# facebookresearch/gtn_applications

Hardware: AMD Instinct MI355X
Metric: utterances/sec fwd+bwd (ctc_benchmark T=1000,C=100,B=128); HBM GB/s vs peak (higher is better)
Workload: dtype f32

## Files before the change

gtn_applications_amd/csrc/ctc_kernels.hip:

```cpp
#include <atomic>
#include <string>
#include <type_traits>

#include "device_common.h"

#ifndef WFL_MITM_STATS
#define WFL_MITM_STATS 0
#endif

namespace wfl {

constexpr float kNegBig = -1.0e30f;
constexpr float kLog2e = 1.4426950408889634f;
constexpr int kBlk = 16;

__device__ __forceinline__ float lse2_b2(float a, float b) {
  const float e = __builtin_amdgcn_exp2f(-fabsf(a - b));
  return vmax(a, b) + __builtin_amdgcn_logf(1.f + e);
}
__device__ __forceinline__ float readlane_f(float v, int lane) {
  return __int_as_float(__builtin_amdgcn_readlane(__float_as_int(v), lane));
}
__device__ __forceinline__ float to_score(float raw) {
  const float v = raw * kLog2e;
// ... 358 lines not shown
  "s_nop 1\n\t"  \
  "v_cndmask_b32_e64 %[t0], %[v1], %[v0], %[m0]\n\t"  \
  "v_cndmask_b32_e64 %[t1], %[v0], %[v1], %[m0]\n\t"  \
  "v_cndmask_b32_e64 %[t2], %[v3], %[v2], %[m0]\n\t"  \
  "v_cndmask_b32_e64 %[t3], %[v2], %[v3], %[m0]\n\t"  \
  OP " %[a0], %[t0], %[t1] quad_perm:[1,0,3,2] row_mask:0xf bank_mask:0xf\n\t"  \
  "v_cndmask_b32_e64 %[t0], %[v5], %[v4], %[m0]\n\t"  \
  "v_cndmask_b32_e64 %[t1], %[v4], %[v5], %[m0]\n\t"  \
  OP " %[a1], %[t2], %[t3] quad_perm:[1,0,3,2] row_mask:0xf bank_mask:0xf\n\t"  \
  "v_cndmask_b32_e64 %[t2], %[v7], %[v6], %[m0]\n\t"  \
  "v_cndmask_b32_e64 %[t3], %[v6], %[v7], %[m0]\n\t"  \
  OP " %[a2], %[t0], %[t1] quad_perm:[1,0,3,2] row_mask:0xf bank_mask:0xf\n\t"  \
  "v_cndmask_b32_e64 %[t0], %[v9], %[v8], %[m0]\n\t"  \
  "v_cndmask_b32_e64 %[t1], %[v8], %[v9], %[m0]\n\t"  \
  OP " %[a3], %[t2], %[t3] quad_perm:[1,0,3,2] row_mask:0xf bank_mask:0xf\n\t"  \
  "v_cndmask_b32_e64 %[t2], %[v11], %[v10], %[m0]\n\t"  \
  "v_cndmask_b32_e64 %[t3], %[v10], %[v11], %[m0]\n\t"  \
  OP " %[a4], %[t0], %[t1] quad_perm:[1,0,3,2] row_mask:0xf bank_mask:0xf\n\t"  \
  "v_cndmask_b32_e64 %[t0], %[v13], %[v12], %[m0]\n\t"  \
  "v_cndmask_b32_e64 %[t1], %[v12], %[v13], %[m0]\n\t"  \
  OP " %[a5], %[t2], %[t3] quad_perm:[1,0,3,2] row_mask:0xf bank_mask:0xf\n\t"  \
  "v_cndmask_b32_e64 %[t2], %[v15], %[v14], %[m0]\n\t"  \
  "v_cndmask_b32_e64 %[t3], %[v14], %[v15], %[m0]\n\t"  \
  OP " %[a6], %[t0], %[t1] quad_perm:[1,0,3,2] row_mask:0xf bank_mask:0xf\n\t"  \
  "s_nop 0\n\t"  \
  OP " %[a7], %[t2], %[t3] quad_perm:[1,0,3,2] row_mask:0xf bank_mask:0xf\n\t"  \
  "v_cndmask_b32_e64 %[t0], %[a1], %[a0], %[m1]\n\t"  \
  "v_cndmask_b32_e64 %[t1], %[a0], %[a1], %[m1]\n\t"  \
  "v_cndmask_b32_e64 %[t2], %[a3], %[a2], %[m1]\n\t"  \
  "v_cndmask_b32_e64 %[t3], %[a2], %[a3], %[m1]\n\t"  \
  OP " %[a0], %[t0], %[t1] quad_perm:[2,3,0,1] row_mask:0xf bank_mask:0xf\n\t"  \
  "v_cndmask_b32_e64 %[t0], %[a5], %[a4], %[m1]\n\t"  \
  "v_cndmask_b32_e64 %[t1], %[a4], %[a5], %[m1]\n\t"  \
  OP " %[a2], %[t2], %[t3] quad_perm:[2,3,0,1] row_mask:0xf bank_mask:0xf\n\t"  \
  "v_cndmask_b32_e64 %[t2], %[a7], %[a6], %[m1]\n\t"  \
  "v_cndmask_b32_e64 %[t3], %[a6], %[a7], %[m1]\n\t"  \
  OP " %[a4], %[t0], %[t1] quad_perm:[2,3,0,1] row_mask:0xf bank_mask:0xf\n\t"  \
  "s_nop 0\n\t"  \
  OP " %[a6], %[t2], %[t3] quad_perm:[2,3,0,1] row_mask:0xf bank_mask:0xf\n\t"  \
  OP " %[a1], %[a0], %[a0] row_ror:12 row_mask:0xf bank_mask:0x5\n\t"  \
  OP " %[a1], %[a2], %[a2] row_ror:12 row_mask:0xf bank_mask:0xa\n\t"  \
  OP " %[a3], %[a4], %[a4] row_ror:12 row_mask:0xf bank_mask:0x5\n\t"  \
  OP " %[a3], %[a6], %[a6] row_ror:12 row_mask:0xf bank_mask:0xa\n\t"  \
  "s_nop 1\n\t"  \
  OP " %[a0], %[a1], %[a1] row_ror:8 row_mask:0xf bank_mask:0x3\n\t"  \
  OP " %[a0], %[a3], %[a3] row_ror:8 row_mask:0xf bank_mask:0xc"
template <bool MAX>
__device__ __forceinline__ float fold16(const float (&v)[16], int lane) {
  float a0, a1, a2, a3, a4, a5, a6, a7, t0, t1, t2, t3;
  const unsigned long long m0 = 0xaaaaaaaaaaaaaaaaull, m1 = 0xccccccccccccccccull;
#define WFL_FOLD16_OPERANDS                                                                                             \
  : [a0] "=&v"(a0), [a1] "=&v"(a1), [a2] "=&v"(a2), [a3] "=&v"(a3), [a4] "=&v"(a4), [a5] "=&v"(a5), [a6] "=&v"(a6),    \
    [a7] "=&v"(a7), [t0] "=&v"(t0), [t1] "=&v"(t1), [t2] "=&v"(t2), [t3] "=&v"(t3)                                      \
  : [v0] "v"(v[0]), [v1] "v"(v[1]), [v2] "v"(v[2]), [v3] "v"(v[3]), [v4] "v"(v[4]), [v5] "v"(v[5]), [v6] "v"(v[6]),    \
    [v7] "v"(v[7]), [v8] "v"(v[8]), [v9] "v"(v[9]), [v10] "v"(v[10]), [v11] "v"(v[11]), [v12] "v"(v[12]),              \
    [v13] "v"(v[13]), [v14] "v"(v[14]), [v15] "v"(v[15]), [m0] "s"(m0), [m1] "s"(m1)
  if (MAX)
    asm(WFL_FOLD16_BODY("v_max_f32_dpp") WFL_FOLD16_OPERANDS);
  else
    asm(WFL_FOLD16_BODY("v_add_f32_dpp") WFL_FOLD16_OPERANDS);
#undef WFL_FOLD16_OPERANDS
  typedef unsigned v2u __attribute__((ext_vector_type(2)));
  v2u sw = __builtin_amdgcn_permlane16_swap(__float_as_uint(a0), __float_as_uint(a0), false, false);
  float t = MAX ? vmax(__uint_as_float(sw.x), __uint_as_float(sw.y)) : __uint_as_float(sw.x) + __uint_as_float(sw.y);
  sw = __builtin_amdgcn_permlane32_swap(__float_as_uint(t), __float_as_uint(t), false, false);
  t = MAX ? vmax(__uint_as_float(sw.x), __uint_as_float(sw.y)) : __uint_as_float(sw.x) + __uint_as_float(sw.y);
  return t;
}
__device__ __forceinline__ float fold16_sum(const float (&v)[16], int lane) { return fold16<false>(v, lane); }

typedef __attribute__((address_space(3))) int lds_int_t;
__device__ __forceinline__ int lds_peek(const int* p) { return *(const volatile lds_int_t*)(const lds_int_t*)p; }
__device__ __forceinline__ void lds_post(int* p, int v) {
  asm volatile("" ::: "memory");
  *(volatile lds_int_t*)(lds_int_t*)p = v;
}

#define WFL_FRAME(P, PH, TT, TL, TH, F, FY)                                   \
  "v_pk_mul_f32 v[6:7], " F ", %[G]\n\t"                                      \
  "v_pk_mul_f32 " TT ", " F ", " P " op_sel_hi:[1,0]\n\t"                     \
  "v_fmac_f32_dpp " TL ", " PH ", v6 wave_shr:1 row_mask:0xf bank_mask:0xf\n\t" \
  "v_fmac_f32_dpp " TH ", " PH ", v7 wave_shr:1 row_mask:0xf bank_mask:0xf\n\t" \
  "v_fmac_f32 " TH ", " FY ", " PH "\n\t"

__device__ __forceinline__ void lsm_seed_rows(float* rows, const float* __restrict__ xsrc, int n, int C, float lse_blk,
                                              float cf_row, int lane) {
  const int total = n * C;
  const unsigned magic = (unsigned)((0x100000000ull + (unsigned)C - 1) / (unsigned)C);
  auto seed = [&](float xv, float l) {
    const float e = __expf((xv == xv ? xv : WFL_NEG_INF) - l);
    return l > WFL_NEG_INF ? -cf_row * e : 0.f;
  };
  constexpr int U = 8;
  if ((C & 3) == 0 && (((uintptr_t)xsrc) & 15) == 0) {
    const int n4 = total >> 2;
    for (int i0 = lane; i0 < n4; i0 += 64 * U) {
      float4 v[U];
      float l[U];
#pragma unroll
      for (int u = 0; u < U; ++u) {
        const int i = min(i0 + 64 * u, n4 - 1);
        v[u] = ((const float4*)xsrc)[i];
        l[u] = __shfl(lse_blk, (int)__umulhi((unsigned)i * 4u, magic), 64);
      }
#pragma unroll
      for (int u = 0; u < U; ++u) {
        const int i = i0 + 64 * u;
        if (i < n4) ((float4*)rows)[i] = float4{seed(v[u].x, l[u]), seed(v[u].y, l[u]), seed(v[u].z, l[u]), seed(v[u].w, l[u])};
      }
    }
  } else {
    for (int i0 = lane; i0 < total; i0 += 64 * U) {
      float v[U], l[U];
#pragma unroll
      for (int u = 0; u < U; ++u) {
        const int i = min(i0 + 64 * u, total - 1);
        v[u] = xsrc[i];
        l[u] = __shfl(lse_blk, (int)__umulhi((unsigned)i, magic), 64);
      }
#pragma unroll
      for (int u = 0; u < U; ++u) {
        const int i = i0 + 64 * u;
        if (i < total) rows[i] = seed(v[u], l[u]);
      }
    }
  }
}

constexpr int kCS = 65;
constexpr int kCTileBytes = kBlk * kCS * 4;
__host__ __device__ __forceinline__ size_t compact_wave_bytes(int C) { return (size_t)kCTileBytes + ((C + 15) & ~15); }
__device__ __forceinline__ void compact_init(float* tile, unsigned char* cmap, int C, int lane) {
  for (int i = lane; i < kBlk * kCS; i += 64) tile[i] = 0.f;
  for (int i = lane; i < ((C + 15) & ~15) / 4; i += 64) ((unsigned int*)cmap)[i] = 0x40404040u;
}
__device__ __forceinline__ void compact_expand(const float* tile, const unsigned char* cmap, float* __restrict__ dst,
                                               const float* __restrict__ xsrc, float lse_blk, int n, int C, float cf,
                                               bool alive, bool soft, int lane) {
  auto softterm = [&](float xv, float l) { return l > WFL_NEG_INF ? cf * __expf((xv == xv ? xv : WFL_NEG_INF) - l) : 0.f; };
  typedef float f4u __attribute__((ext_vector_type(4), aligned(4)));
  const int c4n = C >> 2;
#pragma unroll 2
  for (int j = 0; j < n; ++j) {
    const float l = soft ? readlane_f(lse_blk, j) : 0.f;
    const float* tr = tile + j * kCS;
    float* drow = dst + (int64_t)j * C;
    const float* xr = xsrc + (int64_t)j * C;
    for (int c4 = lane; c4 < c4n; c4 += 64) {
      const unsigned m4 = alive ? ((const unsigned int*)cmap)[c4] : 0x40404040u;
      f4u o = {tr[m4 & 255u], tr[(m4 >> 8) & 255u], tr[(m4 >> 16) & 255u], tr[m4 >> 24]};
      if (soft) {
        const f4u xv = *reinterpret_cast<const f4u*>(xr + 4 * c4);
        o.x -= softterm(xv.x, l), o.y -= softterm(xv.y, l), o.z -= softterm(xv.z, l), o.w -= softterm(xv.w, l);
      }
      *reinterpret_cast<f4u*>(drow + 4 * c4) = o;
    }
    const int c = 4 * c4n + lane;
    if (c < C) {
      float v = tr[alive ? (int)cmap[c] : 64];
      if (soft) v -= softterm(xr[c], l);
      drow[c] = v;
    }
  }
}

template <bool PIPE, bool LSM = false, bool COMPACT = false>
// ... 1129 lines not shown
```

gtn_applications_amd/csrc/ctc_mitm.h:

```cpp
#pragma once

#ifndef WFL_MITM_ABL
#define WFL_MITM_ABL 0
#endif
#ifndef WFL_MITM_STORE
#define WFL_MITM_STORE 2
#endif
#ifndef WFL_MITM_CLAMP_EVERY
#define WFL_MITM_CLAMP_EVERY 1
#endif
#ifndef WFL_MITM_LEAN
#define WFL_MITM_LEAN 1
#endif
#ifndef WFL_MITM_LSM_ROWS
#define WFL_MITM_LSM_ROWS 8
#endif
constexpr int kLsmRows = WFL_MITM_LSM_ROWS;
#ifndef WFL_MITM_STATS
#define WFL_MITM_STATS 0
#endif

constexpr int kMSpinDefault = 1 << 24;
constexpr int kMaxCouple = 100;
constexpr int kMTile = 128;
// ... 29 lines not shown
      default: role = 4, idx = 7; break;
    }
  }
};
template <>
struct MitmK<8> {
  static constexpr int kSlots = 5, kPSlots = 3;
  static constexpr int kStagers = 2, kEmitters = 3, kWaves = 8;
  __device__ static __forceinline__ void role(int wave, int& role, int& idx) {
    switch (wave) {
      case 0: role = 0, idx = 0; break;
      case 4: role = 2, idx = 0; break;
      case 1: role = 3, idx = 0; break;
      case 2: role = 1, idx = 0; break;
      case 3: role = 1, idx = 1; break;
      case 5: role = 4, idx = 0; break;
      case 6: role = 4, idx = 1; break;
      default: role = 4, idx = 2; break;
    }
  }
};

typedef float mv4f __attribute__((ext_vector_type(4)));
template <class K>
struct MitmLds {
  mv4f ring[K::kSlots][kBlk / 2][64];
  float4 pck[K::kPSlots][64];
  float4 ck[K::kSlots][64];
  float fref[K::kSlots][kBlk];
  double offc[K::kSlots];
  double poff[K::kPSlots];
  double offtot;
  int staged[K::kSlots];
  int pready[K::kPSlots];
  int egrab[K::kSlots];
  int pgrab[K::kPSlots];
  double zref;
  int zready;
  int enext;
  int chainpos;
  int ckpos;
  int ckdone;
  int offdone;
  int cmap_ready;
  int abort;
#if WFL_MITM_STATS
  long long blk_t[64];
#endif
};


template <class K>
__device__ __forceinline__ void mitm_give_up(const CtcArgs& a, const CtcWs& w, MitmLds<K>& S) {
  if ((threadIdx.x & 63) == 0) {
    __hip_atomic_fetch_or((int32_t*)(a.ws + w.perr), 1, __ATOMIC_RELAXED, __HIP_MEMORY_SCOPE_AGENT);
    coherent_store64(a.ws + w.suspect, a.token);
  }
  lds_post(&S.abort, 1);
  asm volatile("s_waitcnt vmcnt(0) lgkmcnt(0)" ::: "memory");
  __builtin_amdgcn_endpgm();
}
template <class K>
__device__ __forceinline__ bool mitm_waited_out(const CtcArgs& a, MitmLds<K>& S, int spin) {
  return spin > a.spin || ((spin & 255) == 255 && lds_peek(&S.abort) != 0);
}

__host__ __device__ inline int mitm_first_emitted(int NB, int dir) { return dir == 0 ? NB / 2 : NB - NB / 2; }
__device__ __forceinline__ unsigned long long* mitm_pub(const CtcArgs& a, const CtcWs& w, int b, int dir, int NB) {
  return (unsigned long long*)(a.ws + w.ck) + (int64_t)(b * 2 + dir) * (NB + 1) * a.P;
}

#if WFL_MITM_STATS
#define MITM_T0() const long long _t0 = clock64()
#define MITM_ACC(var) var += clock64() - _t0
#else
#define MITM_T0()
#define MITM_ACC(var)
#endif

typedef float mv2f __attribute__((ext_vector_type(2)));

template <class K, int DIR, bool FULL, bool WIDE, bool LSM = false>
__device__ __forceinline__ void ctc_mitm_emit_block(const mv2f (&F)[kBlk], mv2f sa, int ea, float4 pk, float rsum, double off_sum,
                                                    MitmLds<K>& S, bool first,
                                                    int cnt, float cf, float g, float gs, bool skipn, bool owner, bool adder,
                                                    int lane, float* rows, const unsigned char* cmap, int ycol, int blank, int C, long long* zmm,
                                                    int32_t* zcnt, unsigned long long* suspect, unsigned long long suspect_token,
                                                    int32_t* perr, int spin_bound, float* __restrict__ dst, long long* st_part,
                                                    const float* __restrict__ xsrc = nullptr, float lse_rows = 0.f) {
#if WFL_MITM_STATS
  const long long st_e0 = clock64();
#endif
  const int eb = __float_as_int(pk.z);
  mv2f pa[kBlk];
  const mv2f G = {g, gs};
#pragma unroll
  for (int j = 0; j < kBlk; ++j) {
    if (FULL || j < cnt) {
      const mv2f t = F[j] * G;
      const mv2f o = F[j] * mv2f{sa.x, sa.x};
      float ox = o.x, oy = o.y;
      fmac2_shr1(ox, oy, sa.y, t.x, t.y);
      oy = fmaf(F[j].y, sa.y, oy);
      sa = mv2f{ox, oy};
    }
    pa[j] = sa;
  }
#if WFL_MITM_STATS
  {
    const long long now = __builtin_amdgcn_readfirstlane(__float_as_int(sa.x)) * 0 + clock64();
    st_part[0] += now - st_e0;
  }
#endif
  float bb = pk.x, bl = pk.y;
  float Kn = 0.f;
  bool alive;
  double zk = -1.0e300;
  const int sx = ea + eb;
  if (first) {
    const int eb_next = __builtin_amdgcn_update_dpp(eb, eb, 0x130, 0xf, 0xf, false);
    const float h = lane == 63 ? 0.f : ldexpf(1.f, min(max(eb_next - eb, -200), 100));
    const float hs = skipn ? h : 0.f;
    const float tb0 = bb + bl;
    float tl0 = bl;
    fmac2_shl1(tl0, bb, bl, h, hs);
    const float v = sa.x * tb0 + sa.y * tl0;
    const int own = v > 0.f ? sx + __builtin_amdgcn_frexp_expf(v) : kEmptyE;
    const int E = __builtin_amdgcn_readlane(wave_prefix_max_i(own), 63);
    const float term = v > 0.f ? ldexpf(v, max(sx - E, -200)) : 0.f;
    const float Zm = wave_all_sum(term);
    alive = Zm > 0.f && Zm < 3.0e38f && E > kEmptyE;
    if (alive) Kn = cf * ldexpf(__builtin_amdgcn_rcpf(Zm), min(max(sx - E, -200), 100));
    zk = alive ? off_sum + (double)E + (double)__builtin_amdgcn_logf(Zm) + (double)rsum : -1.0e300;
    if (lane == 0) S.zref = zk;
    lds_post(&S.zready, 1);
    if (lane == 0) {
      const long long zq = z_fixed(zk);
      const long long was_lo = __hip_atomic_fetch_min(zmm, zq, __ATOMIC_RELAXED, __HIP_MEMORY_SCOPE_AGENT);
      const long long was_hi = __hip_atomic_fetch_max(zmm + 1, zq, __ATOMIC_RELAXED, __HIP_MEMORY_SCOPE_AGENT);
      asm volatile("s_waitcnt vmcnt(0)" ::"v"(was_lo), "v"(was_hi) : "memory");
      __hip_atomic_fetch_add(zcnt, 1, __ATOMIC_RELAXED, __HIP_MEMORY_SCOPE_AGENT);
    }
  } else {
    for (int spin = 0; lds_peek(&S.zready) != 1; ++spin) {
      __builtin_amdgcn_s_sleep(2);
      if (spin > spin_bound || ((spin & 255) == 255 && lds_peek(&S.abort) != 0)) {
        if (lane == 0) {
          __hip_atomic_fetch_or(perr, 1, __ATOMIC_RELAXED, __HIP_MEMORY_SCOPE_AGENT);
          coherent_store64(suspect, suspect_token);
        }
        lds_post(&S.abort, 1);
        asm volatile("s_waitcnt vmcnt(0) lgkmcnt(0)" ::: "memory");
        __builtin_amdgcn_endpgm();
      }
    }
    asm volatile("" ::: "memory");
    const double zref = S.zref;
    alive = zref > -1.0e299;
    if (alive) {
      const double D = off_sum + (double)rsum - zref;
      const double Di = floor(D);
      const float frac = __builtin_amdgcn_exp2f((float)(D - Di));
      Kn = cf * frac * ldexpf(1.f, min(max(sx + (int)Di, -200), 100));
    }
  }
#if WFL_MITM_STATS
  st_part[2] += __builtin_amdgcn_readfirstlane(__float_as_int(Kn)) * 0 + clock64() - st_e0;
#endif
  bb *= Kn, bl *= Kn;
  const int ea_next = __builtin_amdgcn_update_dpp(ea, ea, 0x130, 0xf, 0xf, false);
  const float hk = lane == 63 ? 0.f : ldexpf(1.f, min(max(ea - ea_next, -200), 100));
  const float hks = skipn ? hk : 0.f;
  float gbv[kBlk], glv[kBlk];
  mv2f wsum = {0.f, 0.f};
#pragma unroll
  for (int j = 0; j < kBlk; ++j) gbv[j] = 0.f, glv[j] = 0.f;
#pragma unroll
  for (int j = kBlk - 1; j >= 0; --j) {
    if (FULL || j < cnt) {
      const float tb = bb + bl;
      float tl = bl;
      fmac2_shl1(tl, bb, bl, hk, hks);
      const mv2f t = {tb, tl};
      const mv2f gam = pa[j] * t;
      gbv[j] = gam.x, glv[j] = gam.y;
      const float wj = 1.f + (float)j * (1.f / 32.f);
      wsum = gam * mv2f{wj, wj} + wsum;
      const mv2f nb = t * F[j];
      bb = nb.x, bl = nb.y;
    }
  }
#if WFL_MITM_STATS
  st_part[3] += __builtin_amdgcn_readfirstlane(__float_as_int(bb + wsum.x)) * 0 + clock64() - st_e0;
#endif
  constexpr int R0 = DIR == 0 ? 0 : kBlk - 1, RS = DIR == 0 ? 1 : -1;
  const float gtot = fold16_sum(gbv, lane);
  constexpr int TS = WIDE ? kCS : kMTile;
  if (lane < (FULL ? kBlk : cnt)) rows[(R0 + RS * lane) * TS + blank] = gtot;
  float* cell = rows + ycol;
  if (owner) {
#pragma unroll
    for (int j = 0; j < kBlk; ++j)
      if (FULL || j < cnt) cell[(R0 + RS * j) * TS] = glv[j];
  }
  if (adder) {
#pragma unroll
    for (int j = 0; j < kBlk; ++j)
      if (FULL || j < cnt) atomicAdd(&cell[(R0 + RS * j) * TS], glv[j]);
  }
#if WFL_MITM_STATS
  st_part[4] += __builtin_amdgcn_readfirstlane(__float_as_int(gtot)) * 0 + clock64() - st_e0;
#endif
  {
    const float stot = wave_all_sum(wsum.x + wsum.y);
    const int n = FULL ? kBlk : cnt;
    const float want = cf * ((float)n + (float)(n * (n - 1)) * (1.f / 64.f));
    const bool bad_block = alive && !(fabsf(stot - want) <= 2e-4f * fabsf(cf));
    if (bad_block && lane == 0) {
      __hip_atomic_fetch_min(zmm, kZDead, __ATOMIC_RELAXED, __HIP_MEMORY_SCOPE_AGENT);
      coherent_store64(suspect, suspect_token);
    }
  }
#if WFL_MITM_STATS
  const long long st_e1 = clock64();
  st_part[5] += st_e1 - st_e0;
  struct StAcc {
    long long* p;
    long long t;
    __device__ ~StAcc() { p[1] += clock64() - t; }
  } st_acc{st_part, st_e1};
#endif
  const int nrows = FULL ? kBlk : cnt;
  if (WFL_MITM_ABL & 64) return;
  const bool soft = LSM && alive;
  auto softterm = [&](float xv, float l) { return l > WFL_NEG_INF ? cf * __expf((xv == xv ? xv : WFL_NEG_INF) - l) : 0.f; };
  if (WIDE) {
    asm volatile("" ::: "memory");
    if (LSM)
      compact_expand(rows, cmap, dst, xsrc, lse_rows, nrows, C, cf, true, soft, lane);
    else
      compact_expand(rows, cmap, dst, nullptr, 0.f, nrows, C, 1.f, true, false, lane);
    return;
  }
  if ((C & 3) == 0 && (((uintptr_t)dst) & 15) == 0 && (!LSM || (((uintptr_t)xsrc) & 15) == 0)) {
    const int half = lane >> 5, c4 = lane & 31;
    const float4* src = (const float4*)rows + half * (kMTile / 4) + c4;
    float4* out = (float4*)dst + half * (C >> 2) + c4;
    const bool act = c4 < (C >> 2);
    typedef float nf4 __attribute__((ext_vector_type(4)));
    auto store = [&](int r, const nf4& q) {
      if (act && (FULL || r + half < nrows)) {
#if WFL_MITM_STORE == 2
        asm volatile("global_store_dwordx4 %0, %1, off sc0 sc1\n\ts_nop 1" ::"v"(&out[(r >> 1) * (C >> 1)]), "v"(q) : "memory");
#else
        *(nf4*)&out[(r >> 1) * (C >> 1)] = q;
#endif
      }
    };
    if (LSM) {
      int Cx = C;
      asm volatile("" : "+s"(Cx));
#pragma unroll
      for (int h8 = 0; h8 < kBlk; h8 += kLsmRows) {
        nf4 xv[kLsmRows / 2], v[kLsmRows / 2];
#pragma unroll
        for (int r = 0; r < kLsmRows; r += 2)
          xv[r >> 1] = *((const nf4*)(xsrc + (int64_t)min(h8 + r + half, nrows - 1) * Cx) + (act ? c4 : 0));
        asm volatile("" ::: "memory");
#pragma unroll
        for (int r = 0; r < kLsmRows; r += 2) {
          const float4 q = src[((h8 + r) >> 1) * (kMTile / 2)];
          v[r >> 1] = nf4{q.x, q.y, q.z, q.w};
        }
        if (soft) {
#pragma unroll
          for (int r = 0; r < kLsmRows; r += 2) {
            const float l0 = readlane_f(lse_rows, h8 + r), l1 = readlane_f(lse_rows, h8 + r + 1);
            const float l = half ? l1 : l0;
            nf4& o = v[r >> 1];
            const nf4 xq = xv[r >> 1];
            o.x -= softterm(xq.x, l), o.y -= softterm(xq.y, l), o.z -= softterm(xq.z, l), o.w -= softterm(xq.w, l);
          }
        }
#pragma unroll
        for (int r = 0; r < kLsmRows; r += 2) store(h8 + r, v[r >> 1]);
      }
    } else {
      nf4 v[kBlk / 2];
      asm volatile("" ::: "memory");
#pragma unroll
      for (int r = 0; r < kBlk; r += 2) {
        const float4 q = src[(r >> 1) * (kMTile / 2)];
        v[r >> 1] = nf4{q.x, q.y, q.z, q.w};
      }
#pragma unroll
      for (int r = 0; r < kBlk; r += 2) store(r, v[r >> 1]);
    }
  } else {
#ifndef WFL_MITM_NO_UNALIGNED
    int Cs = C;
    asm volatile("" : "+s"(Cs));
#pragma unroll 1
    for (int r = 0; r < nrows; ++r) {
      const float l = LSM ? readlane_f(lse_rows, r) : 0.f;
#pragma unroll 1
      for (int c = lane; c < Cs; c += 64)
        dst[r * Cs + c] = rows[r * kMTile + c] - ((LSM && soft) ? softterm(xsrc[r * Cs + c], l) : 0.f);
    }
#endif
  }
}

template <class K, bool LSM, int DIR, bool WIDE>
__device__ __forceinline__ void ctc_mitm_emitter(const CtcArgs& a, MitmLds<K>& S, int b, int em, int H0, int NB, int L, int y,
                                                 bool skip, bool skipn, bool has_label, const float* __restrict__ coef,
                                                 const float* __restrict__ gout, float* __restrict__ dx, char* smem,
                                                 const CtcWs& w) {
  const int lane = threadIdx.x & 63;
  const int T = a.T, C = a.C;
  constexpr int kTileFloats = WIDE ? kBlk * kCS : kBlk * kMTile;
  float* const tiles = (float*)(smem + ((sizeof(MitmLds<K>) + 15) & ~(size_t)15));
  float* rows = tiles + (size_t)em * kTileFloats;
  unsigned char* cmap = (unsigned char*)(tiles + (size_t)K::kEmitters * kTileFloats);
  for (int i = lane; i < kTileFloats; i += 64) rows[i] = 0.f;
  bool owner = has_label && y != a.blank;
  int first = lane;
  for (int j = 0; j < L; ++j) {
    const bool same = __builtin_amdgcn_readlane(y, j) == y;
    if (same && j < lane) owner = false, first = min(first, j);
  }
  const bool adder = has_label && !owner;
  const int ycol = WIDE ? (has_label ? (y == a.blank ? 63 : first) : 64) : (has_label ? y : 0);
  if (WIDE) {
    if (em == 0) {
      for (int i = lane; i < ((C + 15) & ~15) / 4; i += 64) ((unsigned int*)cmap)[i] = 0x40404040u;
      if (owner) cmap[y] = (unsigned char)lane;
      if (lane == 0) cmap[a.blank] = 63;
      lds_post(&S.cmap_ready, 1);
    } else {
      for (int spin = 0; lds_peek(&S.cmap_ready) != 1; ++spin) {
        __builtin_amdgcn_s_sleep(8);
        if (mitm_waited_out(a, S, spin)) mitm_give_up(a, w, S);
      }
    }
  }
  const float cf = (coef ? coef[b] : 1.f) * (gout ? gout[0] : 1.f);
  long long* zmm = (long long*)(a.ws + w.zloc) + (int64_t)b * 2;
  int32_t* zcnt = (int32_t*)(a.ws + w.zcnt) + b;
  unsigned long long* suspect = (unsigned long long*)(a.ws + w.suspect);
#if WFL_MITM_STATS
  long long st_wait0 = 0, st_wait1 = 0, st_wait2 = 0;
  long long st_part[6] = {0, 0, 0, 0, 0, 0};
  const long long st_begin = clock64();
#else
  long long* st_part = nullptr;
#endif
  auto give_up = [&]() { mitm_give_up(a, w, S); };
  for (;;) {
    int n = 0;
    if (lane == 0) n = atomicAdd(&S.enext, 1);
    n = __builtin_amdgcn_readfirstlane(n);
    if (n >= NB) break;
    const int k = DIR == 0 ? n : NB - 1 - n;
    const int t0 = k * kBlk, cnt = min(kBlk, T - t0);
    const int slot = n % K::kSlots, ps = n % K::kPSlots;
    {
      int spin = 0;
      MITM_T0();
      while (lds_peek(&S.ckdone) < n + 1) {
        __builtin_amdgcn_s_sleep(4);
        if (mitm_waited_out(a, S, ++spin)) give_up();
      }
      MITM_ACC(st_wait0);
    }
    asm volatile("" ::: "memory");
    mv2f F[kBlk];
#pragma unroll
    for (int j = 0; j < kBlk; j += 2) {
      const mv4f f = S.ring[slot][j >> 1][lane];
      F[j] = mv2f{f.x, f.y}, F[j + 1] = mv2f{f.z, f.w};
    }
    const float4 cko = S.ck[slot][lane];
    const int ea = __float_as_int(cko.z);
    const float rr = lane < kBlk ? S.fref[slot][lane] : 0.f;
    const double off_own = S.offc[slot];
    lds_post(&S.egrab[slot], n + 1);
    {
      int spin = 0;
      MITM_T0();
      while (lds_peek(&S.pready[ps]) != n + 1) {
        __builtin_amdgcn_s_sleep(4);
        if (mitm_waited_out(a, S, ++spin)) give_up();
      }
      MITM_ACC(st_wait1);
    }
    asm volatile("" ::: "memory");
    const float4 pk = S.pck[ps][lane];
    const double off_sum = off_own + S.poff[ps];
    lds_post(&S.pgrab[ps], n + 1);
    MITM_T0();
    const float rsum = wave_all_sum(rr);
    const int ea_prev = wave_shr1_i(ea, ea);
    const float g = lane == 0 ? 0.f : ldexpf(1.f, min(max(ea_prev - ea, -200), kMaxCouple));
    const float gs = skip ? g : 0.f;
    float* dst = dx + ((int64_t)b * T + ((WFL_MITM_ABL & 256) ? (t0 & 63) : t0)) * C;
    if (WFL_MITM_ABL & 128) {
      if (n == H0) lds_post(&S.zready, 1);
      continue;
    }
    const float* xsrc = LSM ? a.x + ((int64_t)b * T + t0) * C : nullptr;
    const float lse_rows = LSM ? a.row_lse[(int64_t)b * T + min(t0 + (lane & 15), T - 1)] : 0.f;
    if (cnt == kBlk)
      ctc_mitm_emit_block<K, DIR, true, WIDE, LSM>(F, mv2f{cko.x, cko.y}, ea, pk, rsum, off_sum, S, n == H0, cnt, cf, g, gs, skipn, owner, adder, lane, rows,
                                     cmap, ycol, WIDE ? 63 : a.blank, C, zmm, zcnt, suspect, a.token, (int32_t*)(a.ws + w.perr), a.spin, dst, st_part, xsrc, lse_rows);
    else if (DIR == 0)
      ctc_mitm_emit_block<K, 0, false, WIDE, LSM>(F, mv2f{cko.x, cko.y}, ea, pk, rsum, off_sum, S, n == H0, cnt, cf, g, gs, skipn, owner, adder, lane, rows,
                                    cmap, ycol, WIDE ? 63 : a.blank, C, zmm, zcnt, suspect, a.token, (int32_t*)(a.ws + w.perr), a.spin, dst, st_part, xsrc, lse_rows);
    MITM_ACC(st_wait2);
  }
#if WFL_MITM_STATS
  if (lane == 0) {
    const int wave = threadIdx.x >> 6;
    long long* d = (long long*)(a.ws + w.dbg) + ((int64_t)(b * 2 + DIR) * K::kWaves + wave) * 8;
    unsigned hw;
    asm volatile("s_getreg_b32 %0, hwreg(HW_REG_HW_ID)" : "=s"(hw));
    d[0] = clock64() - st_begin, d[1] = st_wait0, d[2] = st_wait1, d[3] = st_wait2, d[4] = st_part[0], d[5] = hw;
    d[6] = wall_clock64(), d[7] = st_part[1];
    long long* x = (long long*)(a.ws + w.dbg) + 2 * 8 * K::kWaves * (int64_t)a.B + (int64_t)(b * 2 + DIR) * 256 + 128 + em * 8;
    for (int q = 0; q < 6; ++q) x[q] = st_part[q];
  }
#endif
}

template <class K, bool LSM, bool WIDE>
__device__ __forceinline__ void ctc_mitm_body(const CtcArgs& a, int b, int dir, const float* __restrict__ coef,
                                              const float* __restrict__ gout, float* __restrict__ dx, char* smem) {
  MitmLds<K>& S = *reinterpret_cast<MitmLds<K>*>(smem);
#if WFL_MITM_STATS
  const long long st_wall0 = wall_clock64();
#endif
  const int lane = threadIdx.x & 63, wave = __builtin_amdgcn_readfirstlane(threadIdx.x >> 6);
  const int T = a.T, C = a.C, P = a.P;
  const int Lg = P - 1;
  const int64_t og = (int64_t)b * Lg;
  int yg = -1, ygp = -1, ygn = -1;
  const int64_t nlab = a.n_labels;
  if (lane < Lg && og + Lg <= nlab) yg = a.targets[og + (dir == 0 ? lane : Lg - 1 - lane)];
  if (lane >= 1 && lane - 1 < Lg && og + Lg <= nlab) ygp = a.targets[og + (dir == 0 ? lane - 1 : Lg - lane)];
  if (lane + 1 < Lg && og + Lg <= nlab) ygn = a.targets[og + (dir == 0 ? lane + 1 : Lg - 2 - lane)];
  const int64_t o0 = a.offsets[b];
  const int L = (int)(a.offsets[b + 1] - o0);
  int y = -1, yprev = -1, ynext = -1;
  if (o0 == og && L == Lg && og + Lg <= nlab) {
    y = yg, yprev = ygp, ynext = ygn;
  } else {
    if (lane < L) y = a.targets[o0 + (dir == 0 ? lane : L - 1 - lane)];
    if (lane >= 1 && lane - 1 < L) yprev = a.targets[o0 + (dir == 0 ? lane - 1 : L - lane)];
    if (lane + 1 < L) ynext = a.targets[o0 + (dir == 0 ? lane + 1 : L - 2 - lane)];
  }
  const bool has_label = lane < L, has_blank = lane <= L;
  const bool skip = has_label && lane >= 1 && y != yprev;
  const bool skipn = lane + 1 < L && ynext != y;
  const float* xrow = a.x + (int64_t)b * T * C;
  const int col = has_label ? y : a.blank;
  const int Tb = a.xlen ? a.xlen[b] : T;
  const CtcWs w = ctc_ws_layout(a.B, T, P);
  const int NB = ctc_blocks(T);
  const int H0 = mitm_first_emitted(NB, dir);
  if (threadIdx.x < K::kSlots) S.staged[threadIdx.x] = 0;
  if (threadIdx.x < K::kPSlots) S.pready[threadIdx.x] = 0;
  if (threadIdx.x < K::kSlots) S.egrab[threadIdx.x] = 0;
  if (threadIdx.x < K::kPSlots) S.pgrab[threadIdx.x] = 0;
  if (threadIdx.x == 0) S.enext = mitm_first_emitted(ctc_blocks(a.T), dir), S.zready = 0;
  if (threadIdx.x == 0) S.chainpos = 0, S.ckpos = 0, S.ckdone = 0, S.offdone = 0, S.cmap_ready = 0, S.abort = 0;
#if WFL_MITM_STATS
  if (threadIdx.x < 64) S.blk_t[threadIdx.x] = 0;
#endif
  __syncthreads();
  int role, ridx;
  K::role(wave, role, ridx);
  if (role == 5) return;
  if ((WFL_MITM_ABL & 4096) && role == 4) return;
  if ((WFL_MITM_ABL & (16384 | 4096)) && role == 3) return;
#if WFL_MITM_STATS
  long long st_wait0 = 0, st_wait1 = 0, st_wait2 = 0, st_polls = 0;
  const long long st_begin = clock64();
  auto stats_out = [&]() {
    if (lane == 0) {
      long long* d = (long long*)(a.ws + w.dbg) + ((int64_t)(b * 2 + dir) * K::kWaves + wave) * 8;
      unsigned hw;
      asm volatile("s_getreg_b32 %0, hwreg(HW_REG_HW_ID)" : "=s"(hw));
      unsigned xcc;
      asm volatile("s_getreg_b32 %0, hwreg(HW_REG_XCC_ID)" : "=s"(xcc));
      d[0] = clock64() - st_begin, d[1] = st_wait0, d[2] = st_wait1, d[3] = st_wait2, d[4] = st_polls, d[5] = hw | ((long long)(xcc & 15) << 32);
      d[6] = wall_clock64(), d[7] = st_wall0;
    }
  };
#else
  auto stats_out = [&]() {};
// ... 499 lines not shown
```

Before: 3.138 million.

## Fuse alpha and beta recursions into hand-scheduled asm for full non-first blocks

```diff
diff --git a/gtn_applications_amd/csrc/ctc_kernels.hip b/gtn_applications_amd/csrc/ctc_kernels.hip
--- a/gtn_applications_amd/csrc/ctc_kernels.hip
+++ b/gtn_applications_amd/csrc/ctc_kernels.hip
@@ -464,6 +464,21 @@
   "v_fmac_f32_dpp " TL ", " PH ", v6 wave_shr:1 row_mask:0xf bank_mask:0xf\n\t" \
   "v_fmac_f32_dpp " TH ", " PH ", v7 wave_shr:1 row_mask:0xf bank_mask:0xf\n\t" \
   "v_fmac_f32 " TH ", " FY ", " PH "\n\t"
+
+#define WFL_EB_STEP(FK, FKY, PP, PPY, PN, PNX, PNY, MA, MB, TX, TY)                \
+  "v_pk_mul_f32 v[6:7], " FK ", %[G]\n\t"                                          \
+  "v_fma_f32 " TX ", " MA ", " MB ", v5\n\t"                                       \
+  "v_pk_mul_f32 " PN ", " FK ", " PP " op_sel_hi:[1,0]\n\t"                        \
+  "v_mov_b32 " TY ", v5\n\t"                                                       \
+  "v_fmac_f32_dpp " PNX ", " PPY ", v6 wave_shr:1 row_mask:0xf bank_mask:0xf\n\t"  \
+  "v_fmac_f32_dpp " TY ", v4, v12 wave_shl:1 row_mask:0xf bank_mask:0xf\n\t"       \
+  "v_fmac_f32_dpp " PNY ", " PPY ", v7 wave_shr:1 row_mask:0xf bank_mask:0xf\n\t"  \
+  "v_fmac_f32_dpp " TY ", v5, v13 wave_shl:1 row_mask:0xf bank_mask:0xf\n\t"       \
+  "v_fmac_f32 " PNY ", " FKY ", " PPY "\n\t"
+#define WFL_EB_NEXT(TT, FJ) "v_pk_mul_f32 v[4:5], " TT ", " FJ "\n\t"
+#define WFL_EB_GAMMA(OJ, OK, PN)                   \
+  "v_pk_mul_f32 " OJ ", " OJ ", v[8:9]\n\t"        \
+  "v_pk_mul_f32 " OK ", " PN ", " OK "\n\t"
 
 __device__ __forceinline__ void lsm_seed_rows(float* rows, const float* __restrict__ xsrc, int n, int C, float lse_blk,
                                               float cf_row, int lane) {
diff --git a/gtn_applications_amd/csrc/ctc_mitm.h b/gtn_applications_amd/csrc/ctc_mitm.h
--- a/gtn_applications_amd/csrc/ctc_mitm.h
+++ b/gtn_applications_amd/csrc/ctc_mitm.h
@@ -135,7 +135,7 @@
 
 template <class K, int DIR, bool FULL, bool WIDE, bool LSM = false>
 __device__ __forceinline__ void ctc_mitm_emit_block(const mv2f (&F)[kBlk], mv2f sa, int ea, float4 pk, float rsum, double off_sum,
-                                                    MitmLds<K>& S, bool first,
+                                                    MitmLds<K>& S, bool first, double& zref_own, bool& zknown,
                                                     int cnt, float cf, float g, float gs, bool skipn, bool owner, bool adder,
                                                     int lane, float* rows, const unsigned char* cmap, int ycol, int blank, int C, long long* zmm,
                                                     int32_t* zcnt, unsigned long long* suspect, unsigned long long suspect_token,
@@ -145,70 +145,30 @@
   const long long st_e0 = clock64();
 #endif
   const int eb = __float_as_int(pk.z);
-  mv2f pa[kBlk];
   const mv2f G = {g, gs};
-#pragma unroll
-  for (int j = 0; j < kBlk; ++j) {
-    if (FULL || j < cnt) {
-      const mv2f t = F[j] * G;
-      const mv2f o = F[j] * mv2f{sa.x, sa.x};
-      float ox = o.x, oy = o.y;
-      fmac2_shr1(ox, oy, sa.y, t.x, t.y);
-      oy = fmaf(F[j].y, sa.y, oy);
-      sa = mv2f{ox, oy};
-    }
-    pa[j] = sa;
-  }
-#if WFL_MITM_STATS
-  {
-    const long long now = __builtin_amdgcn_readfirstlane(__float_as_int(sa.x)) * 0 + clock64();
-    st_part[0] += now - st_e0;
-  }
-#endif
   float bb = pk.x, bl = pk.y;
   float Kn = 0.f;
   bool alive;
-  double zk = -1.0e300;
   const int sx = ea + eb;
-  if (first) {
-    const int eb_next = __builtin_amdgcn_update_dpp(eb, eb, 0x130, 0xf, 0xf, false);
-    const float h = lane == 63 ? 0.f : ldexpf(1.f, min(max(eb_next - eb, -200), 100));
-    const float hs = skipn ? h : 0.f;
-    const float tb0 = bb + bl;
-    float tl0 = bl;
-    fmac2_shl1(tl0, bb, bl, h, hs);
-    const float v = sa.x * tb0 + sa.y * tl0;
-    const int own = v > 0.f ? sx + __builtin_amdgcn_frexp_expf(v) : kEmptyE;
-    const int E = __builtin_amdgcn_readlane(wave_prefix_max_i(own), 63);
-    const float term = v > 0.f ? ldexpf(v, max(sx - E, -200)) : 0.f;
-    const float Zm = wave_all_sum(term);
-    alive = Zm > 0.f && Zm < 3.0e38f && E > kEmptyE;
-    if (alive) Kn = cf * ldexpf(__builtin_amdgcn_rcpf(Zm), min(max(sx - E, -200), 100));
-    zk = alive ? off_sum + (double)E + (double)__builtin_amdgcn_logf(Zm) + (double)rsum : -1.0e300;
-    if (lane == 0) S.zref = zk;
-    lds_post(&S.zready, 1);
-    if (lane == 0) {
-      const long long zq = z_fixed(zk);
-      const long long was_lo = __hip_atomic_fetch_min(zmm, zq, __ATOMIC_RELAXED, __HIP_MEMORY_SCOPE_AGENT);
-      const long long was_hi = __hip_atomic_fetch_max(zmm + 1, zq, __ATOMIC_RELAXED, __HIP_MEMORY_SCOPE_AGENT);
-      asm volatile("s_waitcnt vmcnt(0)" ::"v"(was_lo), "v"(was_hi) : "memory");
-      __hip_atomic_fetch_add(zcnt, 1, __ATOMIC_RELAXED, __HIP_MEMORY_SCOPE_AGENT);
-    }
-  } else {
-    for (int spin = 0; lds_peek(&S.zready) != 1; ++spin) {
-      __builtin_amdgcn_s_sleep(2);
-      if (spin > spin_bound || ((spin & 255) == 255 && lds_peek(&S.abort) != 0)) {
-        if (lane == 0) {
-          __hip_atomic_fetch_or(perr, 1, __ATOMIC_RELAXED, __HIP_MEMORY_SCOPE_AGENT);
-          coherent_store64(suspect, suspect_token);
-        }
-        lds_post(&S.abort, 1);
-        asm volatile("s_waitcnt vmcnt(0) lgkmcnt(0)" ::: "memory");
-        __builtin_amdgcn_endpgm();
-      }
-    }
-    asm volatile("" ::: "memory");
-    const double zref = S.zref;
+  auto kn_later = [&]() {
+    if (!zknown) {
+      for (int spin = 0; lds_peek(&S.zready) != 1; ++spin) {
+        __builtin_amdgcn_s_sleep(2);
+        if (spin > spin_bound || ((spin & 255) == 255 && lds_peek(&S.abort) != 0)) {
+          if (lane == 0) {
+            __hip_atomic_fetch_or(perr, 1, __ATOMIC_RELAXED, __HIP_MEMORY_SCOPE_AGENT);
+            coherent_store64(suspect, suspect_token);
+          }
+          lds_post(&S.abort, 1);
+          asm volatile("s_waitcnt vmcnt(0) lgkmcnt(0)" ::: "memory");
+          __builtin_amdgcn_endpgm();
+        }
+      }
+      asm volatile("" ::: "memory");
+      zref_own = S.zref;
+      zknown = true;
+    }
+    const double zref = zref_own;
     alive = zref > -1.0e299;
     if (alive) {
       const double D = off_sum + (double)rsum - zref;
@@ -216,36 +176,138 @@
       const float frac = __builtin_amdgcn_exp2f((float)(D - Di));
       Kn = cf * frac * ldexpf(1.f, min(max(sx + (int)Di, -200), 100));
     }
-  }
-#if WFL_MITM_STATS
-  st_part[2] += __builtin_amdgcn_readfirstlane(__float_as_int(Kn)) * 0 + clock64() - st_e0;
-#endif
-  bb *= Kn, bl *= Kn;
+  };
   const int ea_next = __builtin_amdgcn_update_dpp(ea, ea, 0x130, 0xf, 0xf, false);
   const float hk = lane == 63 ? 0.f : ldexpf(1.f, min(max(ea - ea_next, -200), 100));
   const float hks = skipn ? hk : 0.f;
   float gbv[kBlk], glv[kBlk];
   mv2f wsum = {0.f, 0.f};
-#pragma unroll
-  for (int j = 0; j < kBlk; ++j) gbv[j] = 0.f, glv[j] = 0.f;
-#pragma unroll
-  for (int j = kBlk - 1; j >= 0; --j) {
-    if (FULL || j < cnt) {
-      const float tb = bb + bl;
-      float tl = bl;
-      fmac2_shl1(tl, bb, bl, hk, hks);
-      const mv2f t = {tb, tl};
-      const mv2f gam = pa[j] * t;
-      gbv[j] = gam.x, glv[j] = gam.y;
+  if (FULL && !first) {
+    kn_later();
+#if WFL_MITM_STATS
+    st_part[2] += __builtin_amdgcn_readfirstlane(__float_as_int(Kn)) * 0 + clock64() - st_e0;
+#endif
+    mv4f q[kBlk / 2], o[kBlk / 2];
+#pragma unroll
+    for (int i = 0; i < kBlk / 2; ++i) q[i] = mv4f{F[2 * i].x, F[2 * i].y, F[2 * i + 1].x, F[2 * i + 1].y};
+    mv2f B = {bb * Kn, bl * Kn};
+    const mv2f H = {hk, hks};
+    asm volatile(
+        WFL_EB_STEP("v[16:17]", "v17", "v[2:3]", "v3", "v[48:49]", "v48", "v49", "%[PKX]", "%[KN]", "v78", "v79") WFL_EB_NEXT("v[78:79]", "v[46:47]")
+        WFL_EB_STEP("v[18:19]", "v19", "v[48:49]", "v49", "v[50:51]", "v50", "v51", "v46", "v78", "v76", "v77") WFL_EB_NEXT("v[76:77]", "v[44:45]")
+        WFL_EB_STEP("v[20:21]", "v21", "v[50:51]", "v51", "v[52:53]", "v52", "v53", "v44", "v76", "v74", "v75") WFL_EB_NEXT("v[74:75]", "v[42:43]")
+        WFL_EB_STEP("v[22:23]", "v23", "v[52:53]", "v53", "v[54:55]", "v54", "v55", "v42", "v74", "v72", "v73") WFL_EB_NEXT("v[72:73]", "v[40:41]")
+        WFL_EB_STEP("v[24:25]", "v25", "v[54:55]", "v55", "v[56:57]", "v56", "v57", "v40", "v72", "v70", "v71") WFL_EB_NEXT("v[70:71]", "v[38:39]")
+        WFL_EB_STEP("v[26:27]", "v27", "v[56:57]", "v57", "v[58:59]", "v58", "v59", "v38", "v70", "v68", "v69") WFL_EB_NEXT("v[68:69]", "v[36:37]")
+        WFL_EB_STEP("v[28:29]", "v29", "v[58:59]", "v59", "v[60:61]", "v60", "v61", "v36", "v68", "v66", "v67") WFL_EB_NEXT("v[66:67]", "v[34:35]")
+        WFL_EB_STEP("v[30:31]", "v31", "v[60:61]", "v61", "v[62:63]", "v62", "v63", "v34", "v66", "v64", "v65") WFL_EB_NEXT("v[64:65]", "v[32:33]")
+        WFL_EB_STEP("v[32:33]", "v33", "v[62:63]", "v63", "v[2:3]", "v2", "v3", "v32", "v64", "v8", "v9") WFL_EB_NEXT("v[8:9]", "v[30:31]")
+        WFL_EB_GAMMA("v[62:63]", "v[64:65]", "v[2:3]")
+        WFL_EB_STEP("v[34:35]", "v35", "v[2:3]", "v3", "v[10:11]", "v10", "v11", "v30", "v8", "v8", "v9") WFL_EB_NEXT("v[8:9]", "v[28:29]")
+        WFL_EB_GAMMA("v[60:61]", "v[66:67]", "v[10:11]")
+        WFL_EB_STEP("v[36:37]", "v37", "v[10:11]", "v11", "v[2:3]", "v2", "v3", "v28", "v8", "v8", "v9") WFL_EB_NEXT("v[8:9]", "v[26:27]")
+        WFL_EB_GAMMA("v[58:59]", "v[68:69]", "v[2:3]")
+        WFL_EB_STEP("v[38:39]", "v39", "v[2:3]", "v3", "v[10:11]", "v10", "v11", "v26", "v8", "v8", "v9") WFL_EB_NEXT("v[8:9]", "v[24:25]")
+        WFL_EB_GAMMA("v[56:57]", "v[70:71]", "v[10:11]")
+        WFL_EB_STEP("v[40:41]", "v41", "v[10:11]", "v11", "v[2:3]", "v2", "v3", "v24", "v8", "v8", "v9") WFL_EB_NEXT("v[8:9]", "v[22:23]")
+        WFL_EB_GAMMA("v[54:55]", "v[72:73]", "v[2:3]")
+        WFL_EB_STEP("v[42:43]", "v43", "v[2:3]", "v3", "v[10:11]", "v10", "v11", "v22", "v8", "v8", "v9") WFL_EB_NEXT("v[8:9]", "v[20:21]")
+        WFL_EB_GAMMA("v[52:53]", "v[74:75]", "v[10:11]")
+        WFL_EB_STEP("v[44:45]", "v45", "v[10:11]", "v11", "v[2:3]", "v2", "v3", "v20", "v8", "v8", "v9") WFL_EB_NEXT("v[8:9]", "v[18:19]")
+        WFL_EB_GAMMA("v[50:51]", "v[76:77]", "v[2:3]")
+        WFL_EB_STEP("v[46:47]", "v47", "v[2:3]", "v3", "v[10:11]", "v10", "v11", "v18", "v8", "v8", "v9")
+        WFL_EB_GAMMA("v[48:49]", "v[78:79]", "v[10:11]")
+        : "+{v[2:3]}"(sa), "+{v[4:5]}"(B), "=&{v[48:51]}"(o[0]), "=&{v[52:55]}"(o[1]), "=&{v[56:59]}"(o[2]), "=&{v[60:63]}"(o[3]),
+          "=&{v[64:67]}"(o[4]), "=&{v[68:71]}"(o[5]), "=&{v[72:75]}"(o[6]), "=&{v[76:79]}"(o[7])
+        : "{v[16:19]}"(q[0]), "{v[20:23]}"(q[1]), "{v[24:27]}"(q[2]), "{v[28:31]}"(q[3]), "{v[32:35]}"(q[4]), "{v[36:39]}"(q[5]),
+          "{v[40:43]}"(q[6]), "{v[44:47]}"(q[7]), "{v[12:13]}"(H), [G] "v"(G), [PKX] "v"(bb), [KN] "v"(Kn)
+        : "v6", "v7", "v8", "v9", "v10", "v11");
+#pragma unroll
+    for (int i = 0; i < kBlk / 2; ++i) gbv[2 * i] = o[i].x, glv[2 * i] = o[i].y, gbv[2 * i + 1] = o[i].z, glv[2 * i + 1] = o[i].w;
+#pragma unroll
+    for (int j = kBlk - 1; j >= 0; --j) {
       const float wj = 1.f + (float)j * (1.f / 32.f);
-      wsum = gam * mv2f{wj, wj} + wsum;
-      const mv2f nb = t * F[j];
-      bb = nb.x, bl = nb.y;
-    }
-  }
-#if WFL_MITM_STATS
-  st_part[3] += __builtin_amdgcn_readfirstlane(__float_as_int(bb + wsum.x)) * 0 + clock64() - st_e0;
-#endif
+      wsum = mv2f{gbv[j], glv[j]} * mv2f{wj, wj} + wsum;
+    }
+#if WFL_MITM_STATS
+    {
+      const long long now = __builtin_amdgcn_readfirstlane(__float_as_int(gbv[0] + wsum.x)) * 0 + clock64();
+      st_part[0] += now - st_e0, st_part[3] += now - st_e0;
+    }
+#endif
+  } else {
+    mv2f pa[kBlk];
+#pragma unroll
+    for (int j = 0; j < kBlk; ++j) {
+      if (FULL || j < cnt) {
+        const mv2f t = F[j] * G;
+        const mv2f o = F[j] * mv2f{sa.x, sa.x};
+        float ox = o.x, oy = o.y;
+        fmac2_shr1(ox, oy, sa.y, t.x, t.y);
+        oy = fmaf(F[j].y, sa.y, oy);
+        sa = mv2f{ox, oy};
+      }
+      pa[j] = sa;
+    }
+#if WFL_MITM_STATS
+    {
+      const long long now = __builtin_amdgcn_readfirstlane(__float_as_int(sa.x)) * 0 + clock64();
+      st_part[0] += now - st_e0;
+    }
+#endif
+    double zk = -1.0e300;
+    if (first) {
+      const int eb_next = __builtin_amdgcn_update_dpp(eb, eb, 0x130, 0xf, 0xf, false);
+      const float h = lane == 63 ? 0.f : ldexpf(1.f, min(max(eb_next - eb, -200), 100));
+      const float hs = skipn ? h : 0.f;
+      const float tb0 = bb + bl;
+      float tl0 = bl;
+      fmac2_shl1(tl0, bb, bl, h, hs);
+      const float v = sa.x * tb0 + sa.y * tl0;
+      const int own = v > 0.f ? sx + __builtin_amdgcn_frexp_expf(v) : kEmptyE;
+      const int E = __builtin_amdgcn_readlane(wave_prefix_max_i(own), 63);
+      const float term = v > 0.f ? ldexpf(v, max(sx - E, -200)) : 0.f;
+      const float Zm = wave_all_sum(term);
+      alive = Zm > 0.f && Zm < 3.0e38f && E > kEmptyE;
+      if (alive) Kn = cf * ldexpf(__builtin_amdgcn_rcpf(Zm), min(max(sx - E, -200), 100));
+      zk = alive ? off_sum + (double)E + (double)__builtin_amdgcn_logf(Zm) + (double)rsum : -1.0e300;
+      if (lane == 0) S.zref = zk;
+      lds_post(&S.zready, 1);
+      if (lane == 0) {
+        const long long zq = z_fixed(zk);
+        const long long was_lo = __hip_atomic_fetch_min(zmm, zq, __ATOMIC_RELAXED, __HIP_MEMORY_SCOPE_AGENT);
+        const long long was_hi = __hip_atomic_fetch_max(zmm + 1, zq, __ATOMIC_RELAXED, __HIP_MEMORY_SCOPE_AGENT);
+        asm volatile("s_waitcnt vmcnt(0)" ::"v"(was_lo), "v"(was_hi) : "memory");
+        __hip_atomic_fetch_add(zcnt, 1, __ATOMIC_RELAXED, __HIP_MEMORY_SCOPE_AGENT);
+      }
+    } else {
+      kn_later();
+    }
+#if WFL_MITM_STATS
+    st_part[2] += __builtin_amdgcn_readfirstlane(__float_as_int(Kn)) * 0 + clock64() - st_e0;
+#endif
+    bb *= Kn, bl *= Kn;
+#pragma unroll
+    for (int j = 0; j < kBlk; ++j) gbv[j] = 0.f, glv[j] = 0.f;
+#pragma unroll
+    for (int j = kBlk - 1; j >= 0; --j) {
+      if (FULL || j < cnt) {
+        const float tb = bb + bl;
+        float tl = bl;
+        fmac2_shl1(tl, bb, bl, hk, hks);
+        const mv2f t = {tb, tl};
+        const mv2f gam = pa[j] * t;
+        gbv[j] = gam.x, glv[j] = gam.y;
+        const float wj = 1.f + (float)j * (1.f / 32.f);
+        wsum = gam * mv2f{wj, wj} + wsum;
+        const mv2f nb = t * F[j];
+        bb = nb.x, bl = nb.y;
+      }
+    }
+#if WFL_MITM_STATS
+    st_part[3] += __builtin_amdgcn_readfirstlane(__float_as_int(bb + wsum.x)) * 0 + clock64() - st_e0;
+#endif
+  }
   constexpr int R0 = DIR == 0 ? 0 : kBlk - 1, RS = DIR == 0 ? 1 : -1;
   const float gtot = fold16_sum(gbv, lane);
   constexpr int TS = WIDE ? kCS : kMTile;
@@ -409,6 +471,8 @@
   long long* st_part = nullptr;
 #endif
   auto give_up = [&]() { mitm_give_up(a, w, S); };
+  double zref_own = -1.0e300;
+  bool zknown = false;
   for (;;) {
     int n = 0;
     if (lane == 0) n = atomicAdd(&S.enext, 1);
@@ -464,10 +528,10 @@
     const float* xsrc = LSM ? a.x + ((int64_t)b * T + t0) * C : nullptr;
     const float lse_rows = LSM ? a.row_lse[(int64_t)b * T + min(t0 + (lane & 15), T - 1)] : 0.f;
     if (cnt == kBlk)
-      ctc_mitm_emit_block<K, DIR, true, WIDE, LSM>(F, mv2f{cko.x, cko.y}, ea, pk, rsum, off_sum, S, n == H0, cnt, cf, g, gs, skipn, owner, adder, lane, rows,
+      ctc_mitm_emit_block<K, DIR, true, WIDE, LSM>(F, mv2f{cko.x, cko.y}, ea, pk, rsum, off_sum, S, n == H0, zref_own, zknown, cnt, cf, g, gs, skipn, owner, adder, lane, rows,
                                      cmap, ycol, WIDE ? 63 : a.blank, C, zmm, zcnt, suspect, a.token, (int32_t*)(a.ws + w.perr), a.spin, dst, st_part, xsrc, lse_rows);
     else if (DIR == 0)
-      ctc_mitm_emit_block<K, 0, false, WIDE, LSM>(F, mv2f{cko.x, cko.y}, ea, pk, rsum, off_sum, S, n == H0, cnt, cf, g, gs, skipn, owner, adder, lane, rows,
+      ctc_mitm_emit_block<K, 0, false, WIDE, LSM>(F, mv2f{cko.x, cko.y}, ea, pk, rsum, off_sum, S, n == H0, zref_own, zknown, cnt, cf, g, gs, skipn, owner, adder, lane, rows,
                                     cmap, ycol, WIDE ? 63 : a.blank, C, zmm, zcnt, suspect, a.token, (int32_t*)(a.ws + w.perr), a.spin, dst, st_part, xsrc, lse_rows);
     MITM_ACC(st_wait2);
   }
```

Result: slower. 2.199 million (-29.9%).
